# steventan0110/nFST

Hardware: AMD Instinct MI355X
Metric: lattice-arcs/sec forward-backward (log-Z) (higher is better)
Workload: dtype f32

## Files before the change

nfst_amd/csrc/fb_kernels.h:

```cpp
#pragma once

struct LdsPlan {
  int rows2, v2, v4;
  __host__ __device__ LdsPlan(int max_rows, int vocab)
      : rows2((max_rows + 1) & ~1), v2((vocab + 3) & ~1), v4((vocab + 3) & ~3) {}
  __host__ __device__ int64_t fb_fixed_precise() const {
    return ((int64_t)2 * rows2 + v2) * 16 + (int64_t)v4 * 4 + 2 * kSweepFlags * 4 + 2048;
  }
  __host__ __device__ int64_t bwd_fixed_precise() const { return ((int64_t)rows2 + v2) * 16 + kSweepFlags * 4 + 1024; }
  static __host__ __device__ int64_t sweep_words(int R, int RS) { return (int64_t)R * kSlotWords + (int64_t)RS * kRawWords; }
  __host__ __device__ int64_t fb_bytes(int R, int RS) const {
    return ((int64_t)2 * rows2 + v2) * 8 + (int64_t)v4 * 4 + 2 * sweep_words(R, RS) * 4 + 2 * kSweepFlags * 4 + 1024;
  }
  __host__ __device__ int64_t bwd_bytes(int R, int RS) const {
    return ((int64_t)rows2 + v2) * 8 + sweep_words(R, RS) * 4 + kSweepFlags * 4;
  }
};


template <int NT, class VT>
__device__ __forceinline__ void store_rows(const VT *alpha, const VT *beta, int row_off, int n_rows, int tid,
                                           float *logalpha, float *logbeta, float2 *beta_me) {
  if (!logalpha && !logbeta && !beta_me) return;
  const int r_lo = row_off, r_hi = row_off + n_rows;
// ... 14 lines not shown
  const int n_head = min(v_lo, r_hi) - r_lo;
  const int n_tail = (v_hi >= v_lo) ? r_hi - v_hi : 0;
  for (int k = tid; k < n_head + n_tail; k += NT) {
    const int r = k < n_head ? r_lo + k : v_hi + (k - n_head), i = r - r_lo;
    if (logalpha) out_store4(logalpha + r, me_log32(alpha[i]));
    if (logbeta) out_store4(logbeta + r, me_log32(beta[i]));
    if (beta_me) {
      const float2 bv = me_f2(beta[i]);
      out_store4(reinterpret_cast<float *>(beta_me + r), bv.x);
      out_store4(reinterpret_cast<float *>(beta_me + r) + 1, bv.y);
    }
  }
}

template <int NT, int EXTRA, bool TW = false, bool PREC = false>
__global__ __launch_bounds__(NT) void k_backward(nfst_batch lat, nfst_scores sc, int R, int RS, float *logbeta,
                                                 double *logz64, float *logz32, float2 *beta_me) {
  static_assert(!PREC || TW, "precise flavour: tile waves");
  typedef typename ValOf<PREC>::T VT;
  extern __shared__ float2 lds_raw[];
  VT *lds = reinterpret_cast<VT *>(lds_raw);
  const int b = blockIdx.x, tid = threadIdx.x, lane = tid & 63;
  if (lat.only && lat.only[b] != lat.only_tag) return;
  const float theta_first = tid < lat.vocab ? sc.theta[(size_t)sc.theta_stride * b + tid] : 0.0f;
  const Meta m = load_meta(lat.meta, b);
  const LdsPlan plan(lat.max_rows, lat.vocab);
  VT *beta = lds;
  VT *th = lds + plan.rows2;
  uint32_t *ring = (uint32_t *)(th + plan.v2);
  const Extra ex{lat.weighted ? lat.arc_w : nullptr, sc.arc_scores};
  const int wv = __builtin_amdgcn_readfirstlane(tid >> 6);
  uint32_t *raw = ring + (size_t)R * kSlotWords;
  constexpr int kTwSlot = PREC ? kSlotWordsP : kSlotWords2;
  const int32_t *bwd_perm = lat.bwd_perm + m.bwd_slot_off;
  constexpr bool kSelf = NT != 512;
  constexpr int kAhead = kSelf ? kDmaAheadShared : kDmaAheadDeep;
  constexpr int kNE = kSelf ? 2 : 4, kFirstX = kSelf ? 2 : 4;
  static_assert(!TW || NT == 512, "tile waves: the one-lattice-per-CU flavour");
  if (TW) {
  } else if (kSelf) {
    if (wv == 1) self_start<kAhead>(m.bwd_u, lat.bwd_stream + m.bwd_off, m.bwd_tiles, raw, lane);
  } else if (wv == 2) {
    loader_start(m.bwd_u, lat.bwd_stream + m.bwd_off, m.bwd_tiles, raw, RS, lane);
  }
  const bool x_wave = TW ? (wv == 1 || wv == 2 || wv == 3 || wv == 5) : (EXTRA != 0 && wv >= kFirstX);
  const int x_index = TW ? (wv < 4 ? wv - 1 : 3) : wv - kFirstX;
  WeightWave<8, kNE, EXTRA, TW, PREC> xw8;
  if (x_wave && m.bwd_u == 8) xw8.start_maps(lat.bwd_stream + m.bwd_off, bwd_perm, m.bwd_tiles, ex, x_index, lane);
  for (int i = tid; i < m.n_rows; i += NT) val_set(beta[i], 0.0f, kEZero);
  load_theta(th, sc.theta, sc.theta_stride, b, lat.vocab, tid, NT, theta_first);
  if (x_wave && m.bwd_u == 8) xw8.start_gathers(lane);
  __syncthreads();
  int *flags = (int *)(ring + (TW ? (int64_t)R * kTwSlot : LdsPlan::sweep_words(R, RS)));
  if (tid == 0) {
    val_set(beta[m.sink], 0.5f, 1);
    for (int i = 0; i < kSweepFlags; ++i) flags[i] = 0;
  }
  __syncthreads();
  const bool tw_v2 = TW && m.bwd_wide == 0;
  if (x_wave) {
    run_weights<kNE, EXTRA, TW, PREC>(xw8, m.bwd_u, lat.bwd_stream + m.bwd_off, bwd_perm, m.bwd_tiles, ex, x_index, ring, R, flags,
                                      (const float2 *)th, (const float2 *)beta, tw_v2, lds_addr(flags + kSweepFlags) + lane * (PREC ? 16 : 8), 0u, 0, lane);
  } else if constexpr (TW) {
    if (wv == 0) {
      __builtin_amdgcn_s_setprio(3);
      if constexpr (PREC) tile_sweep2<Sweep64, kNE>(m.bwd_tiles, ring, R, flags, flags + 4, lane);
      else if (tw_v2) tile_sweep2<Sweep32, kNE>(m.bwd_tiles, ring, R, flags, flags + 4, lane);
      else tile_sweep<4, true, kNE>(m.bwd_tiles, ring, R, flags, flags + 4, lane);
      __builtin_amdgcn_s_setprio(0);
    }
  } else if (wv < (kSelf ? 2 : 3))
    run_sweep<EXTRA, kSelf, kAhead, kNE>(wv, m.bwd_u, m.bwd_wide != 0, raw, RS, lat.bwd_stream + m.bwd_off,
              m.bwd_tiles, ring, R, flags, (float2 *)beta, (const float2 *)th, lane);
  __syncthreads();
  if (tid == 0) {
    const double z = me_log64(beta[0]);
    if (logz64) logz64[b] = z;
    if (logz32) logz32[b] = (float)z;
  }
  store_rows<NT, VT>(nullptr, beta, m.row_off, m.n_rows, tid, nullptr, logbeta, beta_me);
}

__device__ __forceinline__ void exp_me_fast(float extra, float &m, int &e) {
  const float x = fminf(fmaxf(extra, -1.0e8f), 9.0e7f);
  const float kf = rintf(x * 1.44269504088896341f);
  float t = fmaf(-kf, 0.693145751953125f, x);
  t = fmaf(-kf, 1.42860682030941723e-6f, t);
  m = __builtin_amdgcn_exp2f(t * 1.44269504088896341f);
  e = (int)kf;
}
__device__ __forceinline__ float arc_posterior(const float2 av, const float2 bv, const float2 tw, float rz,
                                               int ez, bool has_extra, float mx, int ex) {
// ... 321 lines not shown
```

nfst_amd/csrc/tile_format.h:

```cpp
#pragma once

#include <stdint.h>

#if defined(__HIP__)
#define NFST_HD __attribute__((host)) __attribute__((device))
#else
#define NFST_HD
#endif

namespace nfst_tile {

constexpr int64_t kStreamSlack = 512;
constexpr int kArcSpare = 8;
constexpr int kNarrowG = 3, kWideG = 6;
constexpr int kFmtCompact = 8;
constexpr int kCompactLabels = 2048;
constexpr int64_t kMaxOffset = 0x7ffff000;

NFST_HD constexpr int fmt_u(int F) { return F == kFmtCompact ? 4 : F; }
NFST_HD constexpr int fmt_words(int F) { return F == kFmtCompact ? 256 : 64 * (1 + F); }
NFST_HD constexpr int32_t meta_fmt(bool compact, int U, bool wide) { return (compact ? kFmtCompact : U) | ((wide ? 1 : 0) << 8); }
NFST_HD constexpr int meta_code(int32_t w) { return w & 0xff; }
NFST_HD constexpr int meta_wide(int32_t w) { return (w >> 8) & 1; }

// ... 9 lines not shown

NFST_HD constexpr uint32_t rec32(uint32_t state, uint32_t label) { return (state << 3) | (label << 16); }
NFST_HD constexpr uint32_t rec32_state(uint32_t r) { return (r & 0xffffu) >> 3; }
NFST_HD constexpr uint32_t rec32_label(uint32_t r) { return r >> 16; }
NFST_HD constexpr uint32_t rec24(uint32_t state, uint32_t label) { return state | (label << 13); }
NFST_HD constexpr uint32_t rec24_state(uint32_t r) { return r & 0x1fffu; }
NFST_HD constexpr uint32_t rec24_label(uint32_t r) { return (r >> 13) & 0x7ffu; }
NFST_HD constexpr uint32_t rec24_to_32(uint32_t r) { return rec32(rec24_state(r), rec24_label(r)); }
NFST_HD constexpr uint32_t ctl_off8(uint32_t c) { return c & 0xffffu; }
NFST_HD constexpr uint32_t rec32_off8(uint32_t r) { return r & 0xffffu; }
NFST_HD constexpr uint32_t rec32_label8(uint32_t r) { return (r >> 16) << 3; }
NFST_HD constexpr uint32_t rec24_off8(uint32_t r) { return (r << 3) & 0xfff8u; }
NFST_HD constexpr uint32_t rec24_label8(uint32_t r) { return (r >> 10) & 0x3ff8u; }
NFST_HD inline void pack24(const uint32_t (&r)[4], uint32_t &w1, uint32_t &w2, uint32_t &w3) {
  w1 = r[0] | (r[1] << 24);
  w2 = (r[1] >> 8) | (r[2] << 16);
  w3 = (r[2] >> 16) | (r[3] << 8);
}
NFST_HD inline void unpack24(uint32_t w1, uint32_t w2, uint32_t w3, uint32_t (&r)[4]) {
#if defined(__HIP_DEVICE_COMPILE__)
  r[0] = w1; r[1] = __builtin_amdgcn_alignbit(w2, w1, 24); r[2] = __builtin_amdgcn_alignbit(w3, w2, 16); r[3] = w3 >> 8;
#else
  r[0] = w1; r[1] = (w1 >> 24) | (w2 << 8); r[2] = (w2 >> 16) | (w3 << 16); r[3] = w3 >> 8;
#endif
}

NFST_HD inline int ceil_log2(int x) { return x <= 1 ? 0 : 32 - __builtin_clz(x - 1); }
NFST_HD inline int group_cap(int max_g, int U) { return (1 << max_g) * U; }
struct Shape {
  int row, b0, e0;
  int n_part;
  int first;
};
NFST_HD inline int tree_parts(int deg, int max_g, int cap) { return (max_g == kNarrowG && deg > 2 * cap) ? (deg + cap - 1) / cap : 0; }
NFST_HD inline int chain_pieces(int len, int cap) { return len <= cap ? 1 : 1 + (len - 2) / (cap - 1); }
NFST_HD inline int state_passes(const Shape &st, int cap) { return st.n_part ? 1 + chain_pieces(st.n_part, cap) : chain_pieces(st.e0 - st.b0, cap); }
NFST_HD inline int state_pieces(const Shape &st, int cap) { return st.n_part ? st.n_part + chain_pieces(st.n_part, cap) : chain_pieces(st.e0 - st.b0, cap); }
NFST_HD inline int pass_pieces(const Shape &st, int pass) { return st.n_part && pass == 0 ? st.n_part : 1; }

struct Piece {
  int row;
  int begin, end;
  int accum;
  int units;
  int g;
};
// ... 47 lines not shown
```

nfst_amd/csrc/tile_pipeline.h:

```cpp
#pragma once

constexpr int kDmaAheadDeep = 8, kRawSlotsDeep = 12, kDmaAheadShared = 4, kRawSlotsShared = kDmaAheadShared + 1;
constexpr int kRawWords = 64 * (1 + 4);
constexpr int kSlotWords = 64 * (1 + 3 * 4);
constexpr int kSlotWords2 = 1024;
constexpr int kSlotWordsP = 1280;
constexpr int kPreciseTiles = 192;
constexpr int kMaxRing = 12, kMinRing = 3;

template <int STAGES>
__device__ __forceinline__ int seg_max(int Em, int g) { return seg_reduce<STAGES>(Em, g, 6, OpMax{}); }
template <int STAGES>
__device__ __forceinline__ float seg_sum(float M, int g) { return seg_reduce<STAGES>(M, g, 6, OpSum{}); }
template <int STAGES>
__device__ __forceinline__ void seg_reduce_exec(float &M, int &E, uint64_t m0, uint64_t m1, uint64_t m2) {
  static_assert(STAGES == 2 || STAGES == 3, "");
  const int e0 = E;
  int d;
  uint64_t sv;
  if (STAGES == 2) {
    asm volatile(
        "s_mov_b64 %[sv], exec\n\t"
        "s_mov_b64 exec, %[m0]\n\t"
        "s_nop 0\n\t"
// ... 534 lines not shown
    step(t + 1, rbb, tb, ra, ta);
  }
  if (SELF) vm_wait<0>();
}

constexpr int kXNap = 12;
template <int F, int NE, int XM, bool FULL, bool PREC = false>
struct WeightWave {
  static_assert(!PREC || (F == 8 && FULL && XM != 3), "precise flavour: compact tiles, tile waves, extras from HBM / L2");
  static constexpr bool GATHER = XM == 1 || XM == 2, CACHED = XM == 3;
  static constexpr int U = fmt_u(F);
  static constexpr bool BOTH = XM == 2;
  static constexpr int RW = F == 8 ? 4 : (FULL ? 1 : 0) + U;
  struct P { int a[XM != 0 ? U : 1]; uint32_t raw[RW]; };
  struct G { float w[GATHER ? U : 1], s[BOTH ? U : 1]; int a[CACHED ? U : 1]; uint32_t valid; uint32_t raw[RW]; };
  P p0, p1, p2;
  G g0, g1, g2;
  const float *bw, *bs;
  const int32_t *perm;
  const uint32_t *prog_words;
  int n_mine, last, ei;

  __device__ __forceinline__ P ld_tile(int i, int lane) const {
    P p;
    const int t = ei + min(i, max(n_mine - 1, 0)) * NE;
    const int32_t *q = perm + (size_t)t * (64 * U) + lane * U;
    const uint32_t *g = prog_words + (size_t)t * fmt_words(F);
    if (XM == 0) p.a[0] = -1;
    if (U == 4) {
      if (XM != 0) {
        const int4 v = *reinterpret_cast<const int4 *>(q);
        p.a[0] = v.x; p.a[XM != 0 ? 1 : 0] = v.y; p.a[XM != 0 ? 2 : 0] = v.z; p.a[XM != 0 ? 3 : 0] = v.w;
      }
      const uint4 x = *reinterpret_cast<const uint4 *>(g + (F == 8 ? 0 : 64) + lane * 4);
      constexpr int o = (F != 8 && FULL) ? 1 : 0;
      p.raw[o] = x.x; p.raw[o + 1] = x.y; p.raw[o + 2] = x.z; p.raw[o + 3] = x.w;
    } else if (U == 2) {
      if (XM != 0) {
        const int2 v = *reinterpret_cast<const int2 *>(q);
        p.a[0] = v.x; p.a[XM != 0 ? 1 : 0] = v.y;
      }
      const uint2 x = *reinterpret_cast<const uint2 *>(g + 64 + lane * 2);
      constexpr int o = FULL ? 1 : 0;
      p.raw[o] = x.x; p.raw[o + 1] = x.y;
    } else {
      if (XM != 0) p.a[0] = q[0];
      p.raw[FULL ? 1 : 0] = g[64 + lane];
    }
    if (F != 8 && FULL) p.raw[0] = g[lane];
    return p;
// ... 23 lines not shown
    g.valid = 0;
#pragma unroll
    for (int j = 0; j < (XM != 0 ? U : 0); ++j) {
      const int a = max(p.a[j], 0);
      if (GATHER) g.w[j] = bw[a];
      if (BOTH) g.s[j] = bs[a];
      if (CACHED) g.a[j] = a;
      g.valid |= (p.a[j] >= 0 ? 1u : 0u) << j;
    }
#pragma unroll
    for (int j = 0; j < RW; ++j) g.raw[j] = p.raw[j];
    return g;
  }
  __device__ __forceinline__ void start_maps(const uint32_t *prog_, const int32_t *perm_, int n_tiles, const Extra ex, int ei_, int lane) {
    perm = perm_; prog_words = prog_; ei = ei_;
    n_mine = n_tiles > ei ? (n_tiles - ei + NE - 1) / NE : 0;
    last = max(n_tiles - 1, 0);
    bw = ex.arc_w ? ex.arc_w : ex.arc_scores;
    bs = ex.arc_scores;
    if (n_tiles <= 0 || n_mine <= 0) { n_mine = 0; return; }
    p0 = ld_tile(0, lane); p1 = ld_tile(1, lane); p2 = ld_tile(2, lane);
  }
  __device__ __forceinline__ void start_gathers(int lane) {
    if (n_mine <= 0) return;
    g0 = issue(p0);
    p0 = ld_tile(3, lane);
    g1 = issue(p1);
  }
  __device__ __forceinline__ void run(uint32_t *ring, int R, const int *prog, int *xland, const float2 *th_, const float2 *val, bool v2,
                                      uint32_t trash, uint32_t xc_base, int xc_first, int lane) {
    const uint32_t xl_a = lds_addr(xland) + (uint32_t)ei * 4;
    if (n_mine <= 0) {
      if (FULL) *(volatile lds_u32 *)(uintptr_t)xl_a = 0x7fffffffu;
      return;
    }
    constexpr uint32_t SB = FULL ? kSlotWords2 * 4 : 64 * (1 + 3 * U) * 4;
    const uint32_t ring_base = lds_addr(ring), prog_a = lds_addr(prog);
    const uint32_t th_base = lds_addr(th_), val_base = lds_addr(val);
    int prog_seen = 0;
    auto process = [&](int i, const auto &g) {
      const int t = ei + min(i, n_mine - 1) * NE;
      uint32_t ctl, opoff[U], lab8[U];
      unpack(g.raw, ctl, opoff, lab8);
      if constexpr (PREC) {
        double om[U];
        int oe[U];
#pragma unroll
        for (int j = 0; j < U; ++j) {
          const v4u tr = *(const lds_v4u *)(uintptr_t)(th_base + 2 * lab8[j]);
          const double tm = __hiloint2double((int)tr.y, (int)tr.x);
          if constexpr (XM == 0) {
            om[j] = tm;
            oe[j] = (int)tr.z;
          } else {
            const double xs = BOTH ? (double)g.w[GATHER ? j : 0] + (double)g.s[BOTH ? j : 0] : (double)g.w[GATHER ? j : 0];
            const ME64 x = exp_split64(((g.valid >> j) & 1u) ? xs : 0.0);
            om[j] = tm * x.m;
            oe[j] = (int)tr.z + x.e;
          }
        }
        while (__builtin_expect(prog_seen < t - R + 1, 0)) {
          prog_seen = __builtin_amdgcn_readfirstlane(*(const volatile lds_u32 *)(uintptr_t)prog_a);
          if (prog_seen < t - R + 1) { if (R >= 8) __builtin_amdgcn_s_sleep(kXNap); else __builtin_amdgcn_s_sleep(1); }
        }
        asm volatile("" ::: "memory");
        const uint32_t sb = ring_base + (uint32_t)(t % R) * (kSlotWordsP * 4);
        const int gl = (int)((ctl >> 20) & 7u);
        const uint32_t dst = (((int)ctl < 0) ? 2 * (ctl & 0xffffu) + val_base : trash) | (ctl & 0x03f00000u);
        *(lds_v4u *)(uintptr_t)(sb + lane * 16) = v4u{dst, gl > 0 ? 0x3ff00000u : 0u, gl > 1 ? 0x3ff00000u : 0u, gl > 2 ? 0x3ff00000u : 0u};
        *(lds_v4u *)(uintptr_t)(sb + 1024 + lane * 16) = v4u{2 * opoff[0] + val_base, 2 * opoff[1 % U] + val_base, 2 * opoff[2 % U] + val_base, 2 * opoff[3 % U] + val_base};
        *(lds_v4u *)(uintptr_t)(sb + 2048 + lane * 16) = v4u{(uint32_t)__double2loint(om[0]), (uint32_t)__double2hiint(om[0]),
                                                             (uint32_t)__double2loint(om[1 % U]), (uint32_t)__double2hiint(om[1 % U])};
        *(lds_v4u *)(uintptr_t)(sb + 3072 + lane * 16) = v4u{(uint32_t)__double2loint(om[2 % U]), (uint32_t)__double2hiint(om[2 % U]),
                                                             (uint32_t)__double2loint(om[3 % U]), (uint32_t)__double2hiint(om[3 % U])};
        *(lds_v4u *)(uintptr_t)(sb + 4096 + lane * 16) = v4u{(uint32_t)oe[0], (uint32_t)oe[1 % U], (uint32_t)oe[2 % U], (uint32_t)oe[3 % U]};
        asm volatile("" ::: "memory");
        *(volatile lds_u32 *)(uintptr_t)xl_a = (uint32_t)(t + 1);
        return;
      }
      v2f tw[U];
#pragma unroll
      for (int j = 0; j < U; ++j) tw[j] = *(const lds_v2f *)(uintptr_t)(th_base + lab8[j]);
      v2f o[U];
#pragma unroll
      for (int j = 0; j < U; ++j) {
        if (XM == 0) { o[j] = tw[j]; continue; }
        if constexpr (XM != 0) {
          const float xs = CACHED ? *(const __attribute__((address_space(3))) float *)(uintptr_t)(xc_base + (uint32_t)(g.a[CACHED ? j : 0] - xc_first) * 4)
                                  : (BOTH ? g.w[GATHER ? j : 0] + g.s[BOTH ? j : 0] : g.w[GATHER ? j : 0]);
          const ME x = exp_split_nb(((g.valid >> j) & 1u) ? xs : 0.0f);
          o[j] = v2f{tw[j].x * x.m, __int_as_float(__float_as_int(tw[j].y) + x.e)};
        }
      }
      while (__builtin_expect(prog_seen < t - R + 1, 0)) {
        prog_seen = __builtin_amdgcn_readfirstlane(*(const volatile lds_u32 *)(uintptr_t)prog_a);
        if (prog_seen < t - R + 1) { if (R >= 8) __builtin_amdgcn_s_sleep(kXNap); else __builtin_amdgcn_s_sleep(1); }
      }
      asm volatile("" ::: "memory");
      const uint32_t sb = ring_base + (uint32_t)(t % R) * SB;
      if (FULL && v2) {
        const int gl = (int)ctl_g(ctl);
        const uint32_t dst = ctl_leader(ctl) ? ctl_off8(ctl) + val_base : trash;
        *(lds_v4u *)(uintptr_t)(sb + lane * 16) = v4u{dst, gl > 0 ? 0x3f800000u : 0u, gl > 1 ? 0x3f800000u : 0u, gl > 2 ? 0x3f800000u : 0u};
        if (U == 4) {
          *(lds_v4u *)(uintptr_t)(sb + 1024 + lane * 16) = v4u{opoff[0] + val_base, opoff[1 % U] + val_base, opoff[2 % U] + val_base, opoff[3 % U] + val_base};
          *(lds_v4f *)(uintptr_t)(sb + 2048 + lane * 16) = v4f{o[0].x, o[0].y, o[1 % U].x, o[1 % U].y};
          *(lds_v4f *)(uintptr_t)(sb + 3072 + lane * 16) = v4f{o[2 % U].x, o[2 % U].y, o[3 % U].x, o[3 % U].y};
        } else if (U == 2) {
          *(lds_v2u *)(uintptr_t)(sb + 1024 + lane * 8) = v2u{opoff[0] + val_base, opoff[1 % U] + val_base};
          *(lds_v4f *)(uintptr_t)(sb + 2048 + lane * 16) = v4f{o[0].x, o[0].y, o[1 % U].x, o[1 % U].y};
        } else {
          *(lds_u32 *)(uintptr_t)(sb + 1024 + lane * 4) = opoff[0] + val_base;
          *(lds_v2f *)(uintptr_t)(sb + 2048 + lane * 8) = o[0];
        }
        asm volatile("" ::: "memory");
        *(volatile lds_u32 *)(uintptr_t)xl_a = (uint32_t)(t + 1);
        return;
      }
      if (FULL) {
        uint32_t oa[U];
#pragma unroll
        for (int j = 0; j < U; ++j) oa[j] = opoff[j] + val_base;
        *(lds_u32 *)(uintptr_t)(sb + lane * 4) = ctl + val_base;
        if (U == 4) *(lds_v4u *)(uintptr_t)(sb + 256 + lane * 16) = v4u{oa[0], oa[1 % U], oa[2 % U], oa[3 % U]};
        else if (U == 2) *(lds_v2u *)(uintptr_t)(sb + 256 + lane * 8) = v2u{oa[0], oa[1 % U]};
        else *(lds_u32 *)(uintptr_t)(sb + 256 + lane * 4) = oa[0];
      }
      if (U == 4) {
        *(lds_v4f *)(uintptr_t)(sb + 256 + 1024 + lane * 16) = v4f{o[0].x, o[0].y, o[1 % U].x, o[1 % U].y};
        *(lds_v4f *)(uintptr_t)(sb + 256 + 2048 + lane * 16) = v4f{o[2 % U].x, o[2 % U].y, o[3 % U].x, o[3 % U].y};
      } else if (U == 2) {
        *(lds_v4f *)(uintptr_t)(sb + 256 + 512 + lane * 16) = v4f{o[0].x, o[0].y, o[1 % U].x, o[1 % U].y};
      } else {
        *(lds_v2f *)(uintptr_t)(sb + 256 + 256 + lane * 8) = o[0];
      }
      asm volatile("" ::: "memory");
      *(volatile lds_u32 *)(uintptr_t)xl_a = (uint32_t)(t + 1);
    };
#define NFST_X_STEP(PU, GN, PL, GC)  \
    GN = issue(PU);                  \
    PL = ld_tile(i + 4, lane);       \
    process(i, GC);
    for (int i = 0; i < n_mine; i += 3) {
      NFST_X_STEP(p2, g2, p1, g0) ++i;
      NFST_X_STEP(p0, g0, p2, g1) ++i;
      NFST_X_STEP(p1, g1, p0, g2) i -= 2;
    }
#undef NFST_X_STEP
    if (FULL) *(volatile lds_u32 *)(uintptr_t)xl_a = 0x7fffffffu;
  }
};

template <int U>
struct TileDec {
  uint32_t w0;
  uint32_t opa[U];
  v2f tw[U];
};

template <int U>
__device__ __forceinline__ void dec_fetch(uint32_t sb, int lane, TileDec<U> &d) {
  d.w0 = *(const lds_u32 *)(uintptr_t)(sb + lane * 4);
  if (U == 4) {
    const v4u a = *(const lds_v4u *)(uintptr_t)(sb + 256 + lane * 16);
    const v4f p = *(const lds_v4f *)(uintptr_t)(sb + 256 + 1024 + lane * 16);
    const v4f q = *(const lds_v4f *)(uintptr_t)(sb + 256 + 2048 + lane * 16);
    d.opa[0] = a.x; d.opa[1 % U] = a.y; d.opa[2 % U] = a.z; d.opa[3 % U] = a.w;
    d.tw[0] = v2f{p.x, p.y}; d.tw[1 % U] = v2f{p.z, p.w}; d.tw[2 % U] = v2f{q.x, q.y}; d.tw[3 % U] = v2f{q.z, q.w};
  } else if (U == 2) {
    const v2u a = *(const lds_v2u *)(uintptr_t)(sb + 256 + lane * 8);
    const v4f p = *(const lds_v4f *)(uintptr_t)(sb + 256 + 512 + lane * 16);
    d.opa[0] = a.x; d.opa[1 % U] = a.y;
// ... 298 lines not shown
  static __device__ __forceinline__ int math(const Dec &c, const Val (&vv)[4], int ref) { return tile_math3(c, vv, ref); }
};
struct Sweep64 {
  static constexpr uint32_t kSlotBytes = kSlotWordsP * 4;
  typedef Dec2P Dec;
  typedef Rec64 Val;
  static __device__ __forceinline__ void fetch(uint32_t sb, int lane, Dec &d) { dec2p_fetch(sb, lane, d); }
  static __device__ __forceinline__ Val gather(uint32_t a) { return rec64_load(a); }
  static __device__ __forceinline__ int math(const Dec &c, const Val (&vv)[4], int ref) { return tile_math3p(c, vv, ref); }
};

template <typename P, int NEF>
__device__ __forceinline__ void tile_sweep2(int n_tiles, const uint32_t *ring, int R, int *prog, const int *land, int lane, int prof_slot = -1) {
  static_assert(NEF == 4, "four tile waves per sweep");
  (void)prof_slot;
  if (n_tiles <= 0) return;
  constexpr uint32_t SB = P::kSlotBytes;
  const uint32_t ring_base = lds_addr(ring), ring_end = ring_base + (uint32_t)R * SB;
  uint32_t land_a = lds_addr(land), prog_a = lds_addr(prog);
  asm volatile("" : "+v"(land_a), "+v"(prog_a));
  auto flags_now = [&]() { return *(const volatile lds_v4u *)(uintptr_t)land_a; };
  auto margin_x = [](const v4u f) { return min(min((int)f.y - 1, (int)f.z - 2), (int)f.w - 3); };
  auto margin_y = [](const v4u f) { return (int)f.x - 4; };
  auto wait_group = [&](int T, int which) {
    for (;;) {
      const v4u f = flags_now();
      if (__builtin_amdgcn_readfirstlane(which ? margin_y(f) : margin_x(f)) > T) break;
      __builtin_amdgcn_s_sleep(1);
    }
    asm volatile("" ::: "memory");
  };
  while (__builtin_amdgcn_readfirstlane((int)*(const volatile lds_u32 *)(uintptr_t)land_a) <= 0) __builtin_amdgcn_s_sleep(1);
  asm volatile("" ::: "memory");
#ifdef NFST_PROF
  if (prof_slot >= 0) NFST_STAMP(prof_slot);
#endif
  uint32_t gbase = ring_base;
  v4u margin = {0u, 0u, 0u, 0u}, margin1 = {0u, 0u, 0u, 0u};
  int ref = 0;
  int dmax0 = 0;
  typename P::Dec da, db;
  P::fetch(gbase, lane, da);
  asm volatile("" ::: "memory");
#define NFST_S2_STEP(K, CUR, NXT)                                                                          \
  {                                                                                                       \
    typename P::Val vv[4];                                                                                \
    _Pragma("unroll") for (int j = 0; j < 4; ++j) vv[j] = P::gather(CUR.opa[j]);                           \
// ... 15 lines not shown
    asm volatile("" ::: "memory");                                                                        \
    __builtin_amdgcn_sched_barrier(0);                                                                    \
  }
  int T = 0;
  for (; T + 4 <= n_tiles; T += 4) {
    asm volatile("" ::"v"(margin));
    if (__builtin_expect(__builtin_amdgcn_readfirstlane(margin_x(margin)) <= T, 0)) wait_group(T, 0);
    NFST_S2_STEP(0, da, db)
    NFST_S2_STEP(1, db, da)
    NFST_S2_STEP(2, da, db)
    NFST_S2_STEP(3, db, da)
    const int e0 = __builtin_amdgcn_readfirstlane(dmax0);
    ref = __builtin_amdgcn_readfirstlane((e0 > -(1 << 27)) ? e0 + ref : ref);
  }
  if (T < n_tiles) {
    asm volatile("" ::"v"(margin));
    if (__builtin_expect(__builtin_amdgcn_readfirstlane(margin_x(margin)) <= T, 0)) wait_group(T, 0);
    NFST_S2_STEP(0, da, db)
    if (T + 1 < n_tiles) {
      NFST_S2_STEP(1, db, da)
      if (T + 2 < n_tiles) NFST_S2_STEP(2, da, db)
    }
  }
#undef NFST_S2_STEP
}

template <int NE, int XM, bool FULL, bool PREC = false>
__device__ __forceinline__ void run_weights(WeightWave<8, NE, XM, FULL, PREC> &x8, int F, const uint32_t *prog_words, const int32_t *perm,
                                            int n_tiles, const Extra ex, int ei, uint32_t *ring, int R, int *flags,
                                            const float2 *th, const float2 *val, bool v2, uint32_t trash, uint32_t xc_base, int xc_first,
                                            int lane) {
  const int *prog = flags;
  int *xland = flags + 4;
  if constexpr (PREC) {
    x8.run(ring, R, prog, xland, th, val, v2, trash, xc_base, xc_first, lane);
    return;
  }
  if (F == 8 || FULL) {
    x8.run(ring, R, prog, xland, th, val, v2, trash, xc_base, xc_first, lane);
  } else if (F == 4) {
    WeightWave<4, NE, XM, FULL> x;
    x.start_maps(prog_words, perm, n_tiles, ex, ei, lane);
    x.start_gathers(lane);
    x.run(ring, R, prog, xland, th, val, v2, trash, xc_base, xc_first, lane);
  } else if (F == 2) {
    WeightWave<2, NE, XM, FULL> x;
    x.start_maps(prog_words, perm, n_tiles, ex, ei, lane);
    x.start_gathers(lane);
    x.run(ring, R, prog, xland, th, val, v2, trash, xc_base, xc_first, lane);
  } else {
    WeightWave<1, NE, XM, FULL> x;
    x.start_maps(prog_words, perm, n_tiles, ex, ei, lane);
    x.start_gathers(lane);
    x.run(ring, R, prog, xland, th, val, v2, trash, xc_base, xc_first, lane);
  }
}

template <typename VT>
__device__ __forceinline__ void load_theta(VT *th, const float *theta, int64_t stride, int b,
                                           int V, int tid, int nt, float first) {
  const float *t = theta + (size_t)stride * b;
  for (int l = tid; l < V; l += nt) {
    const float s = l == tid ? first : t[l];
    if constexpr (std::is_same<VT, Rec64>::value) {
      const ME64 x = exp_split64((double)s);
      val_set(th[l], x.m, x.e);
    } else {
      const ME x = exp_split(s);
      val_set(th[l], x.m, x.e);
    }
  }
  if (tid == 0) {
    val_set(th[V], 0.0f, kEZero);
    val_set(th[V + 1], 0.5f, 1);
  }
}
```

Measured before the change: 141.1 billion.

## Restructure tile-wave weight producer loop with precomputed addresses and deeper prefetch

Result: faster. 147.9 billion, median of 6 (+4.8%).

```diff
diff --git a/nfst_amd/csrc/fb_kernels.h b/nfst_amd/csrc/fb_kernels.h
--- a/nfst_amd/csrc/fb_kernels.h
+++ b/nfst_amd/csrc/fb_kernels.h
@@ -60,6 +60,7 @@
   VT *lds = reinterpret_cast<VT *>(lds_raw);
   const int b = blockIdx.x, tid = threadIdx.x, lane = tid & 63;
   if (lat.only && lat.only[b] != lat.only_tag) return;
+  if (tid == 0) NFST_STAMP(0);
   const float theta_first = tid < lat.vocab ? sc.theta[(size_t)sc.theta_stride * b + tid] : 0.0f;
   const Meta m = load_meta(lat.meta, b);
   const LdsPlan plan(lat.max_rows, lat.vocab);
@@ -103,9 +104,10 @@
     if (wv == 0) {
       __builtin_amdgcn_s_setprio(3);
       if constexpr (PREC) tile_sweep2<Sweep64, kNE>(m.bwd_tiles, ring, R, flags, flags + 4, lane);
-      else if (tw_v2) tile_sweep2<Sweep32, kNE>(m.bwd_tiles, ring, R, flags, flags + 4, lane);
+      else if (tw_v2) tile_sweep2<Sweep32, kNE>(m.bwd_tiles, ring, R, flags, flags + 4, lane, 5);
       else tile_sweep<4, true, kNE>(m.bwd_tiles, ring, R, flags, flags + 4, lane);
       __builtin_amdgcn_s_setprio(0);
+      NFST_STAMP(2);
     }
   } else if (wv < (kSelf ? 2 : 3))
     run_sweep<EXTRA, kSelf, kAhead, kNE>(wv, m.bwd_u, m.bwd_wide != 0, raw, RS, lat.bwd_stream + m.bwd_off,
diff --git a/nfst_amd/csrc/tile_format.h b/nfst_amd/csrc/tile_format.h
--- a/nfst_amd/csrc/tile_format.h
+++ b/nfst_amd/csrc/tile_format.h
@@ -55,6 +55,21 @@
   r[0] = w1; r[1] = __builtin_amdgcn_alignbit(w2, w1, 24); r[2] = __builtin_amdgcn_alignbit(w3, w2, 16); r[3] = w3 >> 8;
 #else
   r[0] = w1; r[1] = (w1 >> 24) | (w2 << 8); r[2] = (w2 >> 16) | (w3 << 16); r[3] = w3 >> 8;
+#endif
+}
+NFST_HD inline void unpack24_fields(uint32_t w1, uint32_t w2, uint32_t w3, uint32_t (&state)[4], uint32_t (&label)[4]) {
+#if defined(__HIP_DEVICE_COMPILE__)
+#define NFST_BFE(D, X, OFF, W) asm("v_bfe_u32 %0, %1, %2, %3" : "=v"(D) : "v"(X), "n"(OFF), "n"(W))
+  const uint32_t r1 = __builtin_amdgcn_alignbit(w2, w1, 24), r2 = __builtin_amdgcn_alignbit(w3, w2, 16);
+  NFST_BFE(state[0], w1, 0, 13);  NFST_BFE(label[0], w1, 13, 11);
+  NFST_BFE(state[1], r1, 0, 13);  NFST_BFE(label[1], w2, 5, 11);
+  NFST_BFE(state[2], w2, 16, 13); NFST_BFE(label[2], r2, 13, 11);
+  NFST_BFE(state[3], w3, 8, 13);  NFST_BFE(label[3], w3, 21, 11);
+#undef NFST_BFE
+#else
+  uint32_t r[4];
+  unpack24(w1, w2, w3, r);
+  for (int j = 0; j < 4; ++j) { state[j] = rec24_state(r[j]); label[j] = rec24_label(r[j]); }
 #endif
 }
 
diff --git a/nfst_amd/csrc/tile_pipeline.h b/nfst_amd/csrc/tile_pipeline.h
--- a/nfst_amd/csrc/tile_pipeline.h
+++ b/nfst_amd/csrc/tile_pipeline.h
@@ -580,10 +580,12 @@
   int n_mine, last, ei;
 
   __device__ __forceinline__ P ld_tile(int i, int lane) const {
+    const int t = ei + min(i, max(n_mine - 1, 0)) * NE;
+    return ld_at(prog_words + (size_t)t * fmt_words(F), perm + (size_t)t * (64 * U), lane);
+  }
+  __device__ __forceinline__ static P ld_at(const uint32_t *g, const int32_t *qt, int lane) {
     P p;
-    const int t = ei + min(i, max(n_mine - 1, 0)) * NE;
-    const int32_t *q = perm + (size_t)t * (64 * U) + lane * U;
-    const uint32_t *g = prog_words + (size_t)t * fmt_words(F);
+    const int32_t *q = qt + lane * U;
     if (XM == 0) p.a[0] = -1;
     if (U == 4) {
       if (XM != 0) {
@@ -653,110 +655,215 @@
     p0 = ld_tile(0, lane); p1 = ld_tile(1, lane); p2 = ld_tile(2, lane);
   }
   __device__ __forceinline__ void start_gathers(int lane) {
-    if (n_mine <= 0) return;
+    if (n_mine <= 0 || (FULL && XM == 0)) return;
     g0 = issue(p0);
     p0 = ld_tile(3, lane);
     g1 = issue(p1);
   }
-  __device__ __forceinline__ void run(uint32_t *ring, int R, const int *prog, int *xland, const float2 *th_, const float2 *val, bool v2,
-                                      uint32_t trash, uint32_t xc_base, int xc_first, int lane) {
-    const uint32_t xl_a = lds_addr(xland) + (uint32_t)ei * 4;
+  template <class S>
+  __device__ __forceinline__ static void weights32(const S &g, const uint32_t (&tha)[U], uint32_t xc_base, int xc_first, v2f (&o)[U]) {
+    v2f tw[U];
+#pragma unroll
+    for (int j = 0; j < U; ++j) tw[j] = *(const lds_v2f *)(uintptr_t)tha[j];
+#pragma unroll
+    for (int j = 0; j < U; ++j) {
+      if (XM == 0) { o[j] = tw[j]; continue; }
+      if constexpr (XM != 0) {
+        const float xs = CACHED ? *(const __attribute__((address_space(3))) float *)(uintptr_t)(xc_base + (uint32_t)(g.a[CACHED ? j : 0] - xc_first) * 4)
+                                : (BOTH ? g.w[GATHER ? j : 0] + g.s[BOTH ? j : 0] : g.w[GATHER ? j : 0]);
+        const ME x = exp_split_nb(((g.valid >> j) & 1u) ? xs : 0.0f);
+        o[j] = v2f{tw[j].x * x.m, __int_as_float(__float_as_int(tw[j].y) + x.e)};
+      }
+    }
+  }
+  template <bool V2>
+  __device__ __forceinline__ void run_tiles(uint32_t *ring, int R, const int *prog, int *xland, const float2 *th_, const float2 *val,
+                                            uint32_t trash, uint32_t xc_base, int xc_first, int lane) {
+    static_assert(FULL && F == 8 && U == 4 && (V2 || !PREC), "tile waves decode compact programs");
+    uint32_t xl_a = lds_addr(xland) + (uint32_t)ei * 4;
+    if constexpr (XM == 0) asm volatile("" : "+v"(xl_a));
     if (n_mine <= 0) {
-      if (FULL) *(volatile lds_u32 *)(uintptr_t)xl_a = 0x7fffffffu;
+      *(volatile lds_u32 *)(uintptr_t)xl_a = 0x7fffffffu;
       return;
     }
-    constexpr uint32_t SB = FULL ? kSlotWords2 * 4 : 64 * (1 + 3 * U) * 4;
-    const uint32_t ring_base = lds_addr(ring), prog_a = lds_addr(prog);
-    const uint32_t th_base = lds_addr(th_), val_base = lds_addr(val);
-    int prog_seen = 0;
-    auto process = [&](int i, const auto &g) {
-      const int t = ei + min(i, n_mine - 1) * NE;
-      uint32_t ctl, opoff[U], lab8[U];
-      unpack(g.raw, ctl, opoff, lab8);
+    constexpr uint32_t SB = (PREC ? kSlotWordsP : kSlotWords2) * 4;
+    constexpr int SH = PREC ? 4 : 3;
+    constexpr bool kClamp = XM != 0;
+    constexpr int kLoadAhead = XM == 0 ? 3 : 4;
+    const uint32_t prog_a = lds_addr(prog), th_base = lds_addr(th_), val_base = lds_addr(val);
+    const uint32_t ring_bytes = (uint32_t)R * SB, ring_end = lds_addr(ring) + ring_bytes;
+    const uint32_t l16 = (uint32_t)lane * 16;
+    const int t_last = ei + (n_mine - 1) * NE;
+    int t = ei;
+    uint32_t sb = lds_addr(ring) + (uint32_t)ei * SB;
+    constexpr size_t kStep = (size_t)NE * fmt_words(F);
+    const size_t first = (size_t)(ei + (kClamp ? min(kLoadAhead, n_mine - 1) : kLoadAhead) * NE) * fmt_words(F);
+    const uint32_t *gp = prog_words + first, *const gp_last = prog_words + (size_t)t_last * fmt_words(F);
+    const int32_t *qp = perm + first;
+    auto load = [&](P &p) {
+      p = ld_at(gp, qp, lane);
+      const size_t st = !kClamp || gp != gp_last ? kStep : 0;
+      gp += st;
+      qp += st;
+    };
+    struct Dec { v4u h; uint32_t opa[4]; v2f o[PREC ? 1 : 4]; double om[PREC ? 4 : 1]; int oe[PREC ? 4 : 1]; };
+    auto decode = [&](const auto &g) {
+      Dec d;
+      const uint32_t ctl = g.raw[0];
       if constexpr (PREC) {
-        double om[U];
-        int oe[U];
-#pragma unroll
-        for (int j = 0; j < U; ++j) {
-          const v4u tr = *(const lds_v4u *)(uintptr_t)(th_base + 2 * lab8[j]);
+        const int gl = (int)((ctl >> 20) & 7u);
+        const uint32_t dst = (((int)ctl < 0) ? 2 * (ctl & 0xffffu) + val_base : trash) | (ctl & 0x03f00000u);
+        d.h = v4u{dst, gl > 0 ? 0x3ff00000u : 0u, gl > 1 ? 0x3ff00000u : 0u, gl > 2 ? 0x3ff00000u : 0u};
+      } else if constexpr (V2) {
+        const int gl = (int)ctl_g(ctl);
+        const uint32_t dst = ctl_leader(ctl) ? ctl_off8(ctl) + val_base : trash;
+        d.h = v4u{dst, gl > 0 ? 0x3f800000u : 0u, gl > 1 ? 0x3f800000u : 0u, gl > 2 ? 0x3f800000u : 0u};
+      } else {
+        d.h = v4u{ctl + val_base, 0u, 0u, 0u};
+      }
+      if constexpr (XM != 0) {
+      } else if constexpr (PREC || V2) {
+        asm volatile("" ::"v"(d.h));
+      } else {
+        asm volatile("" ::"v"(d.h.x));
+      }
+      uint32_t st[4], lb[4], tha[4];
+      unpack24_fields(g.raw[1], g.raw[2], g.raw[3], st, lb);
+#pragma unroll
+      for (int j = 0; j < 4; ++j) {
+        d.opa[j] = (st[j] << SH) + val_base;
+        tha[j] = (lb[j] << SH) + th_base;
+      }
+      if constexpr (PREC) {
+#pragma unroll
+        for (int j = 0; j < 4; ++j) {
+          const v4u tr = *(const lds_v4u *)(uintptr_t)tha[j];
           const double tm = __hiloint2double((int)tr.y, (int)tr.x);
           if constexpr (XM == 0) {
-            om[j] = tm;
-            oe[j] = (int)tr.z;
+            d.om[j] = tm;
+            d.oe[j] = (int)tr.z;
           } else {
             const double xs = BOTH ? (double)g.w[GATHER ? j : 0] + (double)g.s[BOTH ? j : 0] : (double)g.w[GATHER ? j : 0];
             const ME64 x = exp_split64(((g.valid >> j) & 1u) ? xs : 0.0);
-            om[j] = tm * x.m;
-            oe[j] = (int)tr.z + x.e;
+            d.om[j] = tm * x.m;
+            d.oe[j] = (int)tr.z + x.e;
           }
         }
-        while (__builtin_expect(prog_seen < t - R + 1, 0)) {
+      } else {
+        weights32(g, tha, xc_base, xc_first, d.o);
+      }
+      return d;
+    };
+    int prog_seen = 0;
+    auto publish = [&](const Dec &d) {
+      if (__builtin_expect(prog_seen < t - R + 1, 0)) {
+        for (;;) {
           prog_seen = __builtin_amdgcn_readfirstlane(*(const volatile lds_u32 *)(uintptr_t)prog_a);
-          if (prog_seen < t - R + 1) { if (R >= 8) __builtin_amdgcn_s_sleep(kXNap); else __builtin_amdgcn_s_sleep(1); }
+          if (prog_seen >= t - R + 1) break;
+          if (R >= 8) __builtin_amdgcn_s_sleep(kXNap); else __builtin_amdgcn_s_sleep(1);
         }
-        asm volatile("" ::: "memory");
-        const uint32_t sb = ring_base + (uint32_t)(t % R) * (kSlotWordsP * 4);
-        const int gl = (int)((ctl >> 20) & 7u);
-        const uint32_t dst = (((int)ctl < 0) ? 2 * (ctl & 0xffffu) + val_base : trash) | (ctl & 0x03f00000u);
-        *(lds_v4u *)(uintptr_t)(sb + lane * 16) = v4u{dst, gl > 0 ? 0x3ff00000u : 0u, gl > 1 ? 0x3ff00000u : 0u, gl > 2 ? 0x3ff00000u : 0u};
-        *(lds_v4u *)(uintptr_t)(sb + 1024 + lane * 16) = v4u{2 * opoff[0] + val_base, 2 * opoff[1 % U] + val_base, 2 * opoff[2 % U] + val_base, 2 * opoff[3 % U] + val_base};
-        *(lds_v4u *)(uintptr_t)(sb + 2048 + lane * 16) = v4u{(uint32_t)__double2loint(om[0]), (uint32_t)__double2hiint(om[0]),
-                                                             (uint32_t)__double2loint(om[1 % U]), (uint32_t)__double2hiint(om[1 % U])};
-        *(lds_v4u *)(uintptr_t)(sb + 3072 + lane * 16) = v4u{(uint32_t)__double2loint(om[2 % U]), (uint32_t)__double2hiint(om[2 % U]),
-                                                             (uint32_t)__double2loint(om[3 % U]), (uint32_t)__double2hiint(om[3 % U])};
-        *(lds_v4u *)(uintptr_t)(sb + 4096 + lane * 16) = v4u{(uint32_t)oe[0], (uint32_t)oe[1 % U], (uint32_t)oe[2 % U], (uint32_t)oe[3 % U]};
-        asm volatile("" ::: "memory");
-        *(volatile lds_u32 *)(uintptr_t)xl_a = (uint32_t)(t + 1);
-        return;
-      }
-      v2f tw[U];
-#pragma unroll
-      for (int j = 0; j < U; ++j) tw[j] = *(const lds_v2f *)(uintptr_t)(th_base + lab8[j]);
+      }
+      asm volatile("" ::: "memory");
+      const uint32_t a = sb + l16;
+      if constexpr (PREC) {
+        *(lds_v4u *)(uintptr_t)a = d.h;
+        *(lds_v4u *)(uintptr_t)(a + 1024) = v4u{d.opa[0], d.opa[1], d.opa[2], d.opa[3]};
+        *(lds_v4u *)(uintptr_t)(a + 2048) = v4u{(uint32_t)__double2loint(d.om[0]), (uint32_t)__double2hiint(d.om[0]),
+                                                (uint32_t)__double2loint(d.om[PREC ? 1 : 0]), (uint32_t)__double2hiint(d.om[PREC ? 1 : 0])};
+        *(lds_v4u *)(uintptr_t)(a + 3072) = v4u{(uint32_t)__double2loint(d.om[PREC ? 2 : 0]), (uint32_t)__double2hiint(d.om[PREC ? 2 : 0]),
+                                                (uint32_t)__double2loint(d.om[PREC ? 3 : 0]), (uint32_t)__double2hiint(d.om[PREC ? 3 : 0])};
+        *(lds_v4u *)(uintptr_t)(a + 4096) = v4u{(uint32_t)d.oe[0], (uint32_t)d.oe[PREC ? 1 : 0], (uint32_t)d.oe[PREC ? 2 : 0], (uint32_t)d.oe[PREC ? 3 : 0]};
+      } else {
+        constexpr int J1 = PREC ? 0 : 1, J2 = PREC ? 0 : 2, J3 = PREC ? 0 : 3;
+        const v4f w01 = v4f{d.o[0].x, d.o[0].y, d.o[J1].x, d.o[J1].y}, w23 = v4f{d.o[J2].x, d.o[J2].y, d.o[J3].x, d.o[J3].y};
+        if constexpr (V2) {
+          *(lds_v4u *)(uintptr_t)a = d.h;
+          *(lds_v4u *)(uintptr_t)(a + 1024) = v4u{d.opa[0], d.opa[1], d.opa[2], d.opa[3]};
+          *(lds_v4f *)(uintptr_t)(a + 2048) = w01;
+          *(lds_v4f *)(uintptr_t)(a + 3072) = w23;
+        } else {
+          *(lds_u32 *)(uintptr_t)(sb + (uint32_t)lane * 4) = d.h.x;
+          *(lds_v4u *)(uintptr_t)(a + 256) = v4u{d.opa[0], d.opa[1], d.opa[2], d.opa[3]};
+          *(lds_v4f *)(uintptr_t)(a + 256 + 1024) = w01;
+          *(lds_v4f *)(uintptr_t)(a + 256 + 2048) = w23;
+        }
+      }
+      asm volatile("" ::: "memory");
+      *(volatile lds_u32 *)(uintptr_t)xl_a = (uint32_t)(t + 1);
+      const bool more = !kClamp || t != t_last;
+      t += more ? NE : 0;
+      sb += more ? NE * SB : 0u;
+      sb -= sb >= ring_end ? ring_bytes : 0u;
+    };
+    if constexpr (XM == 0) {
+      uint32_t off[3];
+#pragma unroll
+      for (int k = 0; k < 3; ++k) off[k] = l16 + (uint32_t)(k * kStep * 4);
+      auto load0 = [&](P &p, int k) {
+        asm volatile("" : "+v"(off[k]));
+        const uint4 x = *reinterpret_cast<const uint4 *>(reinterpret_cast<const char *>(gp) + off[k]);
+        p.raw[0] = x.x; p.raw[1] = x.y; p.raw[2] = x.z; p.raw[3] = x.w;
+      };
+#define NFST_X_STEP(PK, K) { const Dec d_ = decode(PK); __builtin_amdgcn_sched_barrier(0); load0(PK, K); publish(d_); }
+      int i = 0;
+      for (; i + 2 + kLoadAhead < n_mine; i += 3) {
+        NFST_X_STEP(p0, 0)
+        NFST_X_STEP(p1, 1)
+        NFST_X_STEP(p2, 2)
+        gp += 3 * kStep;
+      }
+#undef NFST_X_STEP
+      const int left = n_mine - i;
+      {
+        const Dec d = decode(p0);
+        if (left > 3) load0(p0, 0);
+        publish(d);
+      }
+      if (left > 1) {
+        const Dec d = decode(p1);
+        if (left > 4) load0(p1, 1);
+        publish(d);
+      }
+      if (left > 2) publish(decode(p2));
+      if (left > 3) publish(decode(p0));
+      if (left > 4) publish(decode(p1));
+    } else {
+#define NFST_X_STEP(PU, GN, PL, GC)  \
+      GN = issue(PU);                \
+      load(PL);                      \
+      publish(decode(GC));
+      for (int i = 0; i < n_mine; i += 3) {
+        NFST_X_STEP(p2, g2, p1, g0)
+        NFST_X_STEP(p0, g0, p2, g1)
+        NFST_X_STEP(p1, g1, p0, g2)
+      }
+#undef NFST_X_STEP
+    }
+    *(volatile lds_u32 *)(uintptr_t)xl_a = 0x7fffffffu;
+  }
+  __device__ __forceinline__ void run(uint32_t *ring, int R, const int *prog, int *xland, const float2 *th_, uint32_t xc_base, int xc_first,
+                                      int lane) {
+    static_assert(!FULL && !PREC, "tile waves: run_tiles");
+    const uint32_t xl_a = lds_addr(xland) + (uint32_t)ei * 4;
+    if (n_mine <= 0) return;
+    constexpr uint32_t SB = 64 * (1 + 3 * U) * 4;
+    const uint32_t ring_base = lds_addr(ring), prog_a = lds_addr(prog);
+    const uint32_t th_base = lds_addr(th_);
+    int prog_seen = 0;
+    auto process = [&](int i, const G &g) {
+      const int t = ei + min(i, n_mine - 1) * NE;
+      uint32_t ctl, opoff[U], lab8[U], tha[U];
+      unpack(g.raw, ctl, opoff, lab8);
+#pragma unroll
+      for (int j = 0; j < U; ++j) tha[j] = th_base + lab8[j];
       v2f o[U];
-#pragma unroll
-      for (int j = 0; j < U; ++j) {
-        if (XM == 0) { o[j] = tw[j]; continue; }
-        if constexpr (XM != 0) {
-          const float xs = CACHED ? *(const __attribute__((address_space(3))) float *)(uintptr_t)(xc_base + (uint32_t)(g.a[CACHED ? j : 0] - xc_first) * 4)
-                                  : (BOTH ? g.w[GATHER ? j : 0] + g.s[BOTH ? j : 0] : g.w[GATHER ? j : 0]);
-          const ME x = exp_split_nb(((g.valid >> j) & 1u) ? xs : 0.0f);
-          o[j] = v2f{tw[j].x * x.m, __int_as_float(__float_as_int(tw[j].y) + x.e)};
-        }
-      }
+      weights32(g, tha, xc_base, xc_first, o);
       while (__builtin_expect(prog_seen < t - R + 1, 0)) {
         prog_seen = __builtin_amdgcn_readfirstlane(*(const volatile lds_u32 *)(uintptr_t)prog_a);
         if (prog_seen < t - R + 1) { if (R >= 8) __builtin_amdgcn_s_sleep(kXNap); else __builtin_amdgcn_s_sleep(1); }
       }
       asm volatile("" ::: "memory");
       const uint32_t sb = ring_base + (uint32_t)(t % R) * SB;
-      if (FULL && v2) {
-        const int gl = (int)ctl_g(ctl);
-        const uint32_t dst = ctl_leader(ctl) ? ctl_off8(ctl) + val_base : trash;
-        *(lds_v4u *)(uintptr_t)(sb + lane * 16) = v4u{dst, gl > 0 ? 0x3f800000u : 0u, gl > 1 ? 0x3f800000u : 0u, gl > 2 ? 0x3f800000u : 0u};
-        if (U == 4) {
-          *(lds_v4u *)(uintptr_t)(sb + 1024 + lane * 16) = v4u{opoff[0] + val_base, opoff[1 % U] + val_base, opoff[2 % U] + val_base, opoff[3 % U] + val_base};
-          *(lds_v4f *)(uintptr_t)(sb + 2048 + lane * 16) = v4f{o[0].x, o[0].y, o[1 % U].x, o[1 % U].y};
-          *(lds_v4f *)(uintptr_t)(sb + 3072 + lane * 16) = v4f{o[2 % U].x, o[2 % U].y, o[3 % U].x, o[3 % U].y};
-        } else if (U == 2) {
-          *(lds_v2u *)(uintptr_t)(sb + 1024 + lane * 8) = v2u{opoff[0] + val_base, opoff[1 % U] + val_base};
-          *(lds_v4f *)(uintptr_t)(sb + 2048 + lane * 16) = v4f{o[0].x, o[0].y, o[1 % U].x, o[1 % U].y};
-        } else {
-          *(lds_u32 *)(uintptr_t)(sb + 1024 + lane * 4) = opoff[0] + val_base;
-          *(lds_v2f *)(uintptr_t)(sb + 2048 + lane * 8) = o[0];
-        }
-        asm volatile("" ::: "memory");
-        *(volatile lds_u32 *)(uintptr_t)xl_a = (uint32_t)(t + 1);
-        return;
-      }
-      if (FULL) {
-        uint32_t oa[U];
-#pragma unroll
-        for (int j = 0; j < U; ++j) oa[j] = opoff[j] + val_base;
-        *(lds_u32 *)(uintptr_t)(sb + lane * 4) = ctl + val_base;
-        if (U == 4) *(lds_v4u *)(uintptr_t)(sb + 256 + lane * 16) = v4u{oa[0], oa[1 % U], oa[2 % U], oa[3 % U]};
-        else if (U == 2) *(lds_v2u *)(uintptr_t)(sb + 256 + lane * 8) = v2u{oa[0], oa[1 % U]};
-        else *(lds_u32 *)(uintptr_t)(sb + 256 + lane * 4) = oa[0];
-      }
       if (U == 4) {
         *(lds_v4f *)(uintptr_t)(sb + 256 + 1024 + lane * 16) = v4f{o[0].x, o[0].y, o[1 % U].x, o[1 % U].y};
         *(lds_v4f *)(uintptr_t)(sb + 256 + 2048 + lane * 16) = v4f{o[2 % U].x, o[2 % U].y, o[3 % U].x, o[3 % U].y};
@@ -778,7 +885,6 @@
       NFST_X_STEP(p1, g1, p0, g2) i -= 2;
     }
 #undef NFST_X_STEP
-    if (FULL) *(volatile lds_u32 *)(uintptr_t)xl_a = 0x7fffffffu;
   }
 };
 
@@ -1123,7 +1229,13 @@
   auto flags_now = [&]() { return *(const volatile lds_v4u *)(uintptr_t)land_a; };
   auto margin_x = [](const v4u f) { return min(min((int)f.y - 1, (int)f.z - 2), (int)f.w - 3); };
   auto margin_y = [](const v4u f) { return (int)f.x - 4; };
+#ifdef NFST_PROF
+  int prof_waits = 0;
+#endif
   auto wait_group = [&](int T, int which) {
+#ifdef NFST_PROF
+    ++prof_waits;
+#endif
     for (;;) {
       const v4u f = flags_now();
       if (__builtin_amdgcn_readfirstlane(which ? margin_y(f) : margin_x(f)) > T) break;
@@ -1185,6 +1297,9 @@
       if (T + 2 < n_tiles) NFST_S2_STEP(2, da, db)
     }
   }
+#ifdef NFST_PROF
+  if (prof_slot >= 0 && (threadIdx.x & 63) == 0 && blockIdx.x < 4096) fb_prof[blockIdx.x * kProfSlots + prof_slot + 6] = (unsigned long long)prof_waits;
+#endif
 #undef NFST_S2_STEP
 }
 
@@ -1195,27 +1310,27 @@
                                             int lane) {
   const int *prog = flags;
   int *xland = flags + 4;
-  if constexpr (PREC) {
-    x8.run(ring, R, prog, xland, th, val, v2, trash, xc_base, xc_first, lane);
-    return;
-  }
-  if (F == 8 || FULL) {
-    x8.run(ring, R, prog, xland, th, val, v2, trash, xc_base, xc_first, lane);
+  (void)val; (void)v2; (void)trash;
+  if constexpr (FULL) {
+    if (PREC || v2) x8.template run_tiles<true>(ring, R, prog, xland, th, val, trash, xc_base, xc_first, lane);
+    else x8.template run_tiles<PREC>(ring, R, prog, xland, th, val, trash, xc_base, xc_first, lane);
+  } else if (F == 8) {
+    x8.run(ring, R, prog, xland, th, xc_base, xc_first, lane);
   } else if (F == 4) {
     WeightWave<4, NE, XM, FULL> x;
     x.start_maps(prog_words, perm, n_tiles, ex, ei, lane);
     x.start_gathers(lane);
-    x.run(ring, R, prog, xland, th, val, v2, trash, xc_base, xc_first, lane);
+    x.run(ring, R, prog, xland, th, xc_base, xc_first, lane);
   } else if (F == 2) {
     WeightWave<2, NE, XM, FULL> x;
     x.start_maps(prog_words, perm, n_tiles, ex, ei, lane);
     x.start_gathers(lane);
-    x.run(ring, R, prog, xland, th, val, v2, trash, xc_base, xc_first, lane);
+    x.run(ring, R, prog, xland, th, xc_base, xc_first, lane);
   } else {
     WeightWave<1, NE, XM, FULL> x;
     x.start_maps(prog_words, perm, n_tiles, ex, ei, lane);
     x.start_gathers(lane);
-    x.run(ring, R, prog, xland, th, val, v2, trash, xc_base, xc_first, lane);
+    x.run(ring, R, prog, xland, th, xc_base, xc_first, lane);
   }
 }
 
diff --git a/profiles/tune/tile_time.py b/profiles/tune/tile_time.py
--- /dev/null
+++ b/profiles/tune/tile_time.py
@@ -0,0 +1,55 @@
+import ctypes as C, json, os, sys
+sys.path.insert(0, os.path.dirname(os.path.dirname(os.path.dirname(os.path.abspath(__file__)))))
+import numpy as np, torch
+from nfst_amd import ops, synth, _lib
+from nfst_amd.lattice import LatticeBatch
+
+pos = [a for a in sys.argv[1:] if not a.startswith("--")]
+opt = lambda k: sys.argv[sys.argv.index(k) + 1] if k in sys.argv else None
+for k in ("--json", "--tag"):
+    if opt(k) in pos:
+        pos.remove(opt(k))
+B = int(pos[0]) if pos else 256
+rot = int(pos[1]) if len(pos) > 1 else 4
+dev = torch.device("cuda")
+lats = [LatticeBatch.from_synth(synth.bench_batch(B, first_seed=1234 + 100000 * r), device=dev) for r in range(rot)]
+theta = torch.from_numpy(synth.label_scores(1, 256)).to(dev)
+raw = C.CDLL(_lib.LIB_PATH)
+S = 16
+tiles = lats[0].meta_host[:, _lib.META_BWD_TILES].astype(np.int64)
+long_ = tiles >= 0.9 * tiles.max()
+
+
+def stamps(launch):
+    for it in range(10 * rot + 1):
+        launch(it % rot)
+    torch.cuda.synchronize()
+    buf = np.zeros(B * S, np.uint64)
+    assert raw.nfst_prof_read(buf.ctypes.data_as(C.c_void_p), B * S) == 0
+    return buf.reshape(B, S).astype(np.int64)
+
+
+def report(name, t):
+    ns = (t[:, 2] - t[:, 5]) * 10.0 / tiles
+    waits = t[:, 11]
+    r = {"ns_per_tile_median": float(np.median(ns)), "ns_per_tile_min": float(ns.min()), "ns_per_tile_max": float(ns.max()),
+         "ns_per_tile_long_programs_median": float(np.median(ns[long_])), "long_programs": int(long_.sum()),
+         "sweep_us_longest_program": float((t[:, 2] - t[:, 5])[tiles.argmax()] / 100.0),
+         "first_tile_us_after_entry_median": float(np.median(t[:, 5] - t[:, 0]) / 100.0),
+         "wait_group_entries_sum": int(waits.sum()), "wait_group_entries_max": int(waits.max()),
+         "workgroups_that_waited": int((waits > 0).sum()), "wait_group_entries_long_programs_median": float(np.median(waits[long_]))}
+    print(name, json.dumps(r))
+    return r
+
+
+outs = [None] * rot
+def fb(r):
+    outs[r] = ops.forward_backward(lats[r], theta, out=outs[r])
+res = {"lattices": B, "rotate": rot, "beta_tiles": {"min": int(tiles.min()), "median": float(np.median(tiles)), "max": int(tiles.max())},
+       "k_backward": report("k_backward", stamps(lambda r: ops.backward(lats[r], theta))),
+       "k_forward_backward": report("k_forward_backward", stamps(fb))}
+if opt("--json"):
+    path = opt("--json")
+    doc = json.load(open(path)) if os.path.exists(path) else {}
+    doc.setdefault("tile_time", {})[opt("--tag") or "new"] = res
+    json.dump(doc, open(path, "w"), indent=1)
diff --git a/profiles/tune/tile_wave_slots.py b/profiles/tune/tile_wave_slots.py
--- /dev/null
+++ b/profiles/tune/tile_wave_slots.py
@@ -0,0 +1,72 @@
+import collections
+import json
+import os
+import sys
+
+sys.path.insert(0, os.path.dirname(os.path.abspath(__file__)))
+import trip_slots as ts
+
+KERNELS = {
+    "float32_preloaded": ("18k_forward_backwardILi1024ELi0ELb0ELb1ELb0ELb1EE", "k_forward_backward<1024, 0, false, true, false, true>"),
+    "float32_grad_theta": ("18k_forward_backwardILi1024ELi0ELb0ELb1ELb0ELb0EE", "k_forward_backward<1024, 0, false, true, false, false>"),
+    "precise": ("18k_forward_backwardILi1024ELi0ELb0ELb1ELb1ELb0EE", "k_forward_backward<1024, 0, false, true, true, false>"),
+    "extra1": ("18k_forward_backwardILi1024ELi1ELb0ELb1ELb0ELb0EE", "k_forward_backward<1024, 1, false, true, false, false>"),
+    "backward": ("10k_backwardILi512ELi0ELb1ELb0EE", "k_backward<512, 0, true, false>"),
+}
+
+
+def tile_wave_loops(code):
+    out = []
+    for j, i in ts.innermost_loops(code):
+        body = code[j:i + 1]
+        c = ts.classify(body)
+        ops = collections.Counter(op for _, op, _ in body)
+        loads = sum(v for k, v in ops.items() if k.startswith("global_load"))
+        if c["dpp"] == 0 and loads >= 3 and ops["ds_write_b128"] > 0:
+            w128, w32 = ops["ds_write_b128"], ops["ds_write_b32"]
+            name = "both" if w128 > 15 else "narrow" if w32 <= 3 else "wide"
+            out.append((name, c, body))
+    return out
+
+
+def main(argv):
+    args = [a for a in argv if not a.startswith("--")]
+    opt = lambda k: argv[argv.index(k) + 1] if k in argv else None
+    for k in ("--tag", "--json"):
+        if opt(k) in args:
+            args.remove(opt(k))
+    lib = args[0] if args else os.path.join(ts.ROOT, "nfst_amd", "lib", "libnfst_hip.so")
+    fns = ts.functions(ts.disassemble(lib))
+    res_path = lib[:-3] + ".resources.json"
+    res = json.load(open(res_path)) if os.path.exists(res_path) else {}
+    out = {}
+    for tag, (frag, res_name) in KERNELS.items():
+        sym = [s for s in fns if frag in s and not s.endswith(".kd")]
+        if len(sym) != 1:
+            raise SystemExit(f"{tag}: {len(sym)} symbols match {frag}")
+        entry = {}
+        for name, c, body in tile_wave_loops(fns[sym[0]]):
+            c["per_tile"] = round(c["issued"] / 3.0, 2)
+            ops = collections.Counter(op for _, op, _ in body)
+            c["mnemonics"] = {k: v for k, v in sorted(ops.items(), key=lambda kv: -kv[1]) if v > 3}
+            while name in entry:
+                name += "_"
+            entry[name] = c
+            print(tag, name, json.dumps(c))
+            if "--dump" in argv:
+                for a, op, ar in body:
+                    print("  %06x  %s %s" % (a, op, ar))
+        r = next((v for k, v in res.items() if k.split("(")[0].strip() == res_name), None)
+        if r is not None:
+            entry["registers"] = {k: r.get(k) for k in ("vgprs", "agprs", "sgprs", "scratch", "vgpr_spill", "sgpr_spill", "occupancy")}
+        out[tag] = entry
+    if opt("--json"):
+        path = opt("--json")
+        doc = json.load(open(path)) if os.path.exists(path) else {}
+        doc.setdefault("tile_wave_loop", {})[opt("--tag") or "new"] = out
+        json.dump(doc, open(path, "w"), indent=1)
+    return 0
+
+
+if __name__ == "__main__":
+    sys.exit(main(sys.argv[1:]))
```
